# VGLoic/kzg-poly-commit-exploration

Measured on AMD Instinct MI355X. Metric: g1_msm_commitments_per_sec_degree_2^20, higher is better.
Workload: dtype i32 digits (Fp: 13 signed radix-2^30 digits, Montgomery 2^390; Fr: 8 x u32, Montgomery 2^256)

## Files before the change

### include/kzg_mi355x.h

```cpp
#ifndef KZG_MI355X_H
#define KZG_MI355X_H

#include <stddef.h>
#include <stdint.h>

#ifdef __cplusplus
extern "C" {
#endif

typedef struct kzg_ctx kzg_ctx;

#define KZG_ABI_VERSION 4
int kzg_abi_version(void);

typedef enum kzg_status {
    KZG_OK = 0,
    KZG_ERR_DEGREE_TOO_HIGH = -1,
    KZG_ERR_CONSTANT_POLY = -2,
    KZG_ERR_REMAINDER = -3,
    KZG_ERR_INVALID_ARG = -4,
    KZG_ERR_NO_DEVICE = -5,
    KZG_ERR_HIP = -6,
    KZG_ERR_NO_SRS = -7,
    KZG_ERR_BUSY = -8
// ... 478 lines not shown
                   size_t* bad_index );
int kzg_srs_verify_lincomb(kzg_ctx* ctx, const uint64_t* weights, const void* setup_g2, size_t g2_stride_bytes,
                           uint64_t out_a_p1[18], uint64_t out_b_p1[18], int* valid);

int kzg_g2_mul(const uint64_t in_p2[36], const uint8_t scalar_be[32], uint64_t out_p2[36]);
int kzg_srs_verify_update(const uint64_t before_p1[18], const uint64_t after_p1[18], const uint64_t tau_g2[36], int* valid);


typedef struct kzg_kernel_times {
    float digits_ms;
    float scatter_ms;
    float accumulate_ms;
    float reduce_ms;
    float quotient_ms;
    float total_ms;
    uint64_t references;
    float accumulate_events_ms;
    float reserved_;
} kzg_kernel_times;

int kzg_set_timing(kzg_ctx* ctx, int enabled);
int kzg_get_times(kzg_ctx* ctx, int slot, kzg_kernel_times* out);
int kzg_msm_config(const kzg_ctx* ctx, int* digit_bits, int* table_levels, size_t* num_buckets, int* recoding);

#ifdef __cplusplus
}
#endif
#endif
```

### kzg_poly_commit_exploration_amd/__init__.py

```python
import ctypes as C
import os

import numpy as np

__all__ = [
    "Engine", "Scalar", "G1Point", "Polynomial", "Evaluation", "SetupArtifactsGenerator", "KzgError",
    "R_MODULUS", "lib_path", "load_library", "ABI_SYMBOLS", "srs_g2_at", "verify_proof", "verify_proof_batch",
    "verify_points", "KZG_MAX_OPEN_POINTS", "KZG_NTT_MAX_LOG", "KZG_GP_MAX_COLUMNS", "KZG_PQ_MAX_COLUMNS", "KZG_LOGUP_MAX_COLUMNS",
    "KZG_PQ_MAX_LOG_EXT", "KZG_EXTEND_VALUES", "KZG_EXTEND_COEFFS", "domain_root",
    "Circuit", "circuit_verify", "circuit_blinders", "circuit_blinded_sizes", "circuit_proof_size", "circuit_proof_challenges", "circuit_verify_proof",
    "KZG_CIRCUIT_MIN_COLUMNS", "KZG_CIRCUIT_COL_QLIN", "KZG_CIRCUIT_COL_QM", "KZG_CIRCUIT_COL_QC", "KZG_CIRCUIT_COL_SIGMA",
    "KZG_CIRCUIT_COL_L0", "KZG_CIRCUIT_VALUES", "KZG_CIRCUIT_COEFFS", "KZG_CIRCUIT_COSET",
    "KZG_CIRCUIT_COL_TABLE", "KZG_CIRCUIT_COL_QLOOKUP",
    "circuit_lookup_proof_size", "circuit_lookup_proof_challenges", "circuit_lookup_verify_proof",
    "combine_claims", "verify_combined", "KZG_MAX_COMBINE",
    "verify_sets", "KZG_MAX_SETS", "KZG_MAX_SET_POINTS",
    "sha256", "sha256_has_shani", "blob_challenges_bytes",
]

_HERE = os.path.dirname(os.path.abspath(__file__))
R_MODULUS = 0x73EDA753299D7D483339D80809A1D80553BDA402FFFE5BFEFFFFFFFF00000001
_FR_R = 1 << 256
_FR_RINV = pow(_FR_R, -1, R_MODULUS)

KZG_OK = 0
KZG_ERR_DEGREE_TOO_HIGH = -1
KZG_ERR_CONSTANT_POLY = -2
KZG_ERR_REMAINDER = -3
KZG_ERR_INVALID_ARG = -4
KZG_ERR_NO_DEVICE = -5
KZG_ERR_HIP = -6
KZG_ERR_NO_SRS = -7
KZG_ERR_BUSY = -8
KZG_MULTI_REPLICATE_SRS = 1
KZG_ABI_VERSION = 4

ABI_SYMBOLS = [
    "kzg_ctx_create", "kzg_ctx_destroy", "kzg_strerror", "kzg_last_error",
    "kzg_srs_load_g1", "kzg_srs_generate_g1", "kzg_srs_read_g1", "kzg_srs_len",
    "kzg_commit", "kzg_commit_le_bytes", "kzg_open", "kzg_quotient", "kzg_evaluate",
    "kzg_srs_load_affine", "kzg_srs_load_compressed", "kzg_srs_save", "kzg_srs_load_file",
    "kzg_ctx_create_multi", "kzg_ctx_create_multi_ex", "kzg_abi_version", "kzg_commit_batch", "kzg_open_batch", "kzg_num_devices", "kzg_rccl_exchanges", "kzg_num_slots", "kzg_commit_submit", "kzg_open_submit", "kzg_wait",
    "kzg_set_max_batch", "kzg_max_batch", "kzg_commit_batch_submit", "kzg_wait_batch",
    "kzg_open_batch_submit", "kzg_wait_open_batch", "kzg_g1_uncompress",
    "kzg_dev_alloc", "kzg_dev_free", "kzg_dev_upload", "kzg_dev_download",
    "kzg_g1_sum", "kzg_g1_compress", "kzg_srs_g2_at", "kzg_verify_proof", "kzg_verify_proof_batch", "kzg_set_timing", "kzg_get_times", "kzg_msm_config",
    "kzg_open_points", "kzg_open_points_submit", "kzg_quotient_points", "kzg_evaluate_points", "kzg_verify_points",
    "kzg_domain_root", "kzg_ntt", "kzg_ntt_device", "kzg_commit_evaluations", "kzg_commit_evaluations_submit",
    "kzg_open_evaluations", "kzg_cells_and_proofs", "kzg_cells_and_proofs_evaluations", "kzg_quotient_cells",
    "kzg_cells_and_proofs_fk20", "kzg_fk20_prepare", "kzg_g1_dft", "kzg_recover_cells_and_proofs",
    "kzg_verify_cells_batch", "kzg_verify_cells_lincomb",
    "kzg_evaluate_evaluations_batch", "kzg_verify_openings_batch", "kzg_verify_openings_lincomb", "kzg_verify_evaluations_batch",
    "kzg_verify_cells_batch_bytes", "kzg_verify_cells_lincomb_bytes", "kzg_verify_openings_batch_bytes",
    "kzg_verify_openings_lincomb_bytes", "kzg_verify_blobs_batch_bytes", "kzg_g1_uncompress_batch", "kzg_fr_from_bytes_batch",
    "kzg_blobs_to_commitments_bytes", "kzg_blobs_to_cells_and_proofs_bytes", "kzg_recover_cells_and_proofs_bytes",
    "kzg_g1_compress_batch", "kzg_fr_to_bytes_batch",
    "kzg_srs_update", "kzg_srs_verify", "kzg_srs_verify_lincomb", "kzg_g2_mul", "kzg_srs_verify_update",
    "kzg_open_combined", "kzg_open_combined_submit", "kzg_wait_combined", "kzg_get_combine_ms", "kzg_combine_polys",
    "kzg_evaluate_batch_at", "kzg_combine_claims", "kzg_verify_combined",
    "kzg_open_sets", "kzg_open_sets_submit", "kzg_wait_sets", "kzg_quotient_sets", "kzg_verify_sets",
    "kzg_sha256", "kzg_sha256_pieces", "kzg_sha256_has_shani", "kzg_blob_challenges_bytes", "kzg_blobs_open_at_bytes", "kzg_blobs_to_blob_proofs_bytes",
    "kzg_verify_blob_proofs_batch_bytes",
    "kzg_lagrange_prepare", "kzg_lagrange_len", "kzg_lagrange_read_g1", "kzg_lagrange_load_compressed",
    "kzg_srs_load_lagrange_compressed", "kzg_commit_lagrange", "kzg_commit_lagrange_submit", "kzg_commit_lagrange_batch",
    "kzg_open_lagrange", "kzg_open_lagrange_submit", "kzg_quotient_lagrange",
    "kzg_grand_product", "kzg_grand_product_device", "kzg_permutation_product", "kzg_permutation_product_device",
    "kzg_permutation_commit",
    "kzg_logderivative_sum", "kzg_logderivative_sum_device", "kzg_lookup_sum", "kzg_lookup_sum_device", "kzg_lookup_commit",
    "kzg_batch_inverse", "kzg_batch_inverse_device", "kzg_lookup_multiplicities", "kzg_lookup_multiplicities_device",
# ... 102 lines not shown
        "kzg_num_slots": (i, [vp]),
        "kzg_commit_submit": (i, [vp, i, vp, sz]),
        "kzg_open_submit": (i, [vp, i, vp, sz, vp, vp]),
        "kzg_wait": (i, [vp, i, vp]),
        "kzg_set_max_batch": (i, [vp, sz]),
        "kzg_max_batch": (sz, [vp]),
        "kzg_commit_batch_submit": (i, [vp, i, vp, sz, sz, sz]),
        "kzg_wait_batch": (i, [vp, i, vp, sz]),
        "kzg_open_batch_submit": (i, [vp, i, vp, sz, sz, sz, vp, vp]),
        "kzg_wait_open_batch": (i, [vp, i, vp, vp, sz]),
        "kzg_g1_uncompress": (i, [u8p, vp]),
        "kzg_dev_alloc": (i, [vp, sz, C.POINTER(vp)]),
        "kzg_dev_free": (i, [vp, vp]),
        "kzg_dev_upload": (i, [vp, vp, vp, sz]),
        "kzg_dev_download": (i, [vp, vp, vp, sz]),
        "kzg_g1_sum": (i, [vp, sz, vp]),
        "kzg_g1_compress": (i, [vp, vp]),
        "kzg_set_timing": (i, [vp, i]),
        "kzg_get_times": (i, [vp, i, C.POINTER(KernelTimes)]),
        "kzg_srs_g2_at": (i, [u8p, C.c_uint64, vp]),
        "kzg_verify_proof": (i, [vp, vp, vp, vp, vp, C.POINTER(i)]),
        "kzg_verify_proof_batch": (i, [vp, vp, vp, vp, vp, sz, vp]),
        "kzg_msm_config": (i, [vp, C.POINTER(i), C.POINTER(i), C.POINTER(sz), C.POINTER(i)]),
        "kzg_open_points": (i, [vp, vp, sz, vp, vp, sz, vp]),
        "kzg_open_points_submit": (i, [vp, i, vp, sz, vp, vp, sz]),
        "kzg_quotient_points": (i, [vp, vp, sz, vp, vp, sz, vp, C.POINTER(sz)]),
        "kzg_evaluate_points": (i, [vp, vp, sz, vp, sz, vp]),
        "kzg_verify_points": (i, [vp, vp, vp, vp, sz, vp, sz, vp, sz, C.POINTER(i)]),
        "kzg_domain_root": (i, [C.c_uint, vp]),
        "kzg_ntt": (i, [vp, vp, sz, i, vp]),
        "kzg_ntt_device": (i, [vp, vp, vp, sz, i]),
        "kzg_ntt_batch": (i, [vp, vp, sz, sz, sz, i, vp, sz]),
        "kzg_ntt_batch_device": (i, [vp, vp, sz, sz, sz, vp, sz, i]),
        "kzg_ntt_batch_rounds": (i, [vp, sz, sz, C.POINTER(sz)]),
        "kzg_commit_evaluations": (i, [vp, vp, sz, vp]),
        "kzg_commit_evaluations_submit": (i, [vp, i, vp, sz]),
        "kzg_open_evaluations": (i, [vp, vp, sz, vp, vp, vp]),
        "kzg_lagrange_prepare": (i, [vp, C.c_uint]),
        "kzg_lagrange_len": (sz, [vp]),
        "kzg_lagrange_read_g1": (i, [vp, sz, sz, vp]),
        "kzg_lagrange_load_compressed": (i, [vp, vp, sz, C.c_uint, i, C.POINTER(sz), C.POINTER(i)]),
        "kzg_srs_load_lagrange_compressed": (i, [vp, vp, sz, C.c_uint, C.POINTER(sz)]),
        "kzg_commit_lagrange": (i, [vp, vp, sz, vp]),
        "kzg_commit_lagrange_submit": (i, [vp, i, vp, sz]),
        "kzg_commit_lagrange_batch": (i, [vp, vp, sz, sz, sz, vp]),
        "kzg_open_lagrange": (i, [vp, vp, sz, vp, vp, vp]),
# ... 1448 lines not shown
                for i in range(b)]

    def commit_batch_limbs(self, polys):
        polys = [np.ascontiguousarray(p, dtype=np.uint64).reshape(-1, 4) for p in polys]
        n = polys[0].shape[0]
        assert all(p.shape[0] == n for p in polys)
        flat = np.concatenate(polys)
        dptr = self.dev_alloc(flat.nbytes)
        try:
            self.dev_upload(dptr, flat)
            self.commit_batch_submit(0, dptr, n, len(polys))
            return self.wait_batch(0, len(polys))
        finally:
            self.dev_free(dptr)

    def set_timing(self, enabled):
        _check(self._lib.kzg_set_timing(self._h, 1 if enabled else 0))

    def times(self, slot):
        t = KernelTimes()
        _check(self._lib.kzg_get_times(self._h, slot, C.byref(t)))
        return {n: getattr(t, n) for n, _ in KernelTimes._fields_}


class Circuit:

    def __init__(self, engine, handle, n, t, log_ext, key):
        self._eng, self._c = engine, handle
        self.n, self.t, self.log_ext, self.key = n, t, log_ext, key
        self.c = 0
        self.g, self.exponents = 0, None
        self.rho, self.exponents_next = 0, None

    def close(self):
        if getattr(self, "_c", None) and getattr(self._eng, "_h", None):
            self._eng._pq_check(self._eng._lib.kzg_circuit_destroy(self._eng._h, self._c))
        self._c = None

    def quotient(self, wires, z, alpha, beta, gamma, public_inputs=None, gate=None, n=None, want_coeffs=True, want_commitments=True,
                 engine=None):
        e = self._eng if engine is None else engine
        a, t, stride, n = e._columns(wires, self.n if n is None else n)
        assert t == self.t and n == self.n
        zz = np.ascontiguousarray(z, dtype=np.uint64).reshape(-1, 4)
        assert zz.shape[0] >= n
        N = n << self.log_ext
# ... 692 lines not shown
```

### kzg_poly_commit_exploration_amd/csrc/api.hip

```cpp
#include <hip/hip_runtime.h>
#include <sys/random.h>

#include <algorithm>
#include <atomic>
#include <cerrno>
#include <chrono>
#include <condition_variable>
#include <cstdio>
#include <cstdlib>
#include <cstring>
#include <deque>
#include <functional>
#include <mutex>
#include <new>
#include <string>
#include <thread>
#include <vector>

#include "../../include/kzg_mi355x.h"
#include "engine.h"
#include "host_field.hpp"
#include "host_fr.hpp"
#include "fr30_host.hpp"
#include "host_pairing.hpp"
// ... 103 lines not shown

struct SlotQueue {
    hipStream_t stream = nullptr;
    hipStream_t end = nullptr;
    hipEvent_t ev[8] = {};
    hipEvent_t done = nullptr;
    hipEvent_t sorted_ev = nullptr, accum_ev = nullptr;
    hipEvent_t cmb_ev[2] = {};
    hipEvent_t cells_ev = nullptr;
    hipEvent_t upload_ev = nullptr;
    SlotQueue() = default;
    SlotQueue(const SlotQueue&) = delete;
    SlotQueue& operator=(const SlotQueue&) = delete;
    ~SlotQueue() {
        for (hipEvent_t e : {ev[0], ev[1], ev[2], ev[3], ev[4], ev[5], ev[6], ev[7], cmb_ev[0], cmb_ev[1], cells_ev, upload_ev, done, sorted_ev, accum_ev})
            if (e) hipEventDestroy(e);
    }
};

struct Slot : SlotQueue {
    DevBuf cnt, offs, block_sums, pairs, sorted, buckets;
    DevBuf recoded;
    DevBuf part_a, part_b;
    DevBuf pair_scratch;
    DevBuf heavy_ws;
    DevBuf arena;
    PinnedBuf fin{PinnedBuf::Mapped};
    DevBuf stage;
    DevBuf q;
    DevBuf chunk, block;
    PinnedBuf small{PinnedBuf::Mapped};
    PinnedBuf bsmall{PinnedBuf::Mapped};
    std::vector<uint32_t> open_ys;
    PinnedBuf roots{PinnedBuf::Staged};
    PinnedBuf pvals{PinnedBuf::Mapped};
    DevBuf pblock;
    std::vector<uint32_t> pts_ys;
    size_t pts_nq = 0;
    PinnedBuf ctab{PinnedBuf::Staged};
    PinnedBuf cvals{PinnedBuf::Mapped};
    DevBuf cpart, cin;
    size_t cmb_t = 0;
    float combine_ms = 0;
    PinnedBuf stab{PinnedBuf::Staged}, ssel{PinnedBuf::Staged};
    PinnedBuf svals{PinnedBuf::Mapped};
    DevBuf sg;
// ... 105 lines not shown

struct TmpStream {
    hipStream_t s = nullptr;
    ~TmpStream() { if (s) hipStreamDestroy(s); }
};

int sync_unlocked(kzg_ctx* ctx, std::unique_lock<std::mutex>& lk, hipStream_t st, const char* what) {
    lk.unlock();
    const hipError_t e = hipStreamSynchronize(st);
    lk.lock();
    return e == hipSuccess ? KZG_OK : hip_fail(ctx, what, e);
}
constexpr const char* kCopyCoeffs = "hipMemcpyAsync (coefficients)";
int copy_unlocked(kzg_ctx* ctx, std::unique_lock<std::mutex>& lk, hipStream_t st, void* dst, const void* src, size_t bytes,
                  hipMemcpyKind kind, const char* what) {
    if (!bytes) return KZG_OK;
    lk.unlock();
    const hipError_t e = hipMemcpyAsync(dst, src, bytes, kind, st);
    lk.lock();
    return e == hipSuccess ? KZG_OK : hip_fail(ctx, what, e);
}

void free_slot_msm(Slot& s) {
    for (DevBuf* b : {&s.cnt, &s.offs, &s.block_sums, &s.pairs, &s.recoded, &s.sorted, &s.buckets, &s.part_a, &s.part_b, &s.pair_scratch,
                      &s.heavy_ws, &s.arena})
        b->reset();
    s.fin.reset();
}

int create_stream(kzg_ctx* ctx, hipStream_t* out, bool high) {
    int least = 0, greatest = 0;
    HIP_TRY(ctx, hipDeviceGetStreamPriorityRange(&least, &greatest));
    const char* v = std::getenv("KZG_STREAM_PRIORITIES");
    const bool prio = !(v && v[0] == '0');
    HIP_TRY(ctx, hipStreamCreateWithPriority(out, hipStreamNonBlocking, prio ? (high ? greatest : least) : 0));
    return KZG_OK;
}

int ensure_slot_basics(kzg_ctx* ctx, Slot& s) {
    if (s.stream) return KZG_OK;
    if (!ctx->front_stream) {
        int rc = create_stream(ctx, &ctx->front_stream, false);
        if (rc) return rc;
    }
    if (!ctx->upload_stream) HIP_TRY(ctx, hipStreamCreateWithFlags(&ctx->upload_stream, hipStreamNonBlocking));
    for (auto& e : s.ev)
        if (!e) HIP_TRY(ctx, hipEventCreate(&e));
// ... 85 lines not shown
    const size_t pairs = (size_t)cfg.max_digits * ctx->n * B;
    for (int i = 0; i < kNumSlots; i++) {
        Slot& s = ctx->slots[i];
        {
            int rcb = ensure_slot_basics(ctx, s);
            if (rcb) return rcb;
        }
        if (!s.sorted_ev) {
            HIP_TRY(ctx, hipEventCreateWithFlags(&s.sorted_ev, hipEventDisableTiming));
            HIP_TRY(ctx, hipEventCreateWithFlags(&s.accum_ev, hipEventDisableTiming));
        }
        free_slot_msm(s);
        int rc = s.cnt.reserve(ctx, (size_t)sort_count_entries((uint32_t)B, cfg) * 4 + 64);
        if (rc == KZG_OK) rc = s.offs.reserve(ctx, ((size_t)cfg.nb * B + 1) * 4);
        if (rc == KZG_OK) rc = s.block_sums.reserve(ctx, (size_t)sort_workspace_words() * 4);
        if (rc) return rc;
        HIP_TRY(ctx, hipMemset(s.block_sums.p, 0, (size_t)sort_workspace_zero_words() * 4));
        rc = s.pairs.reserve(ctx, (pairs ? pairs : 1) * 8);
        if (rc == KZG_OK) rc = s.recoded.reserve(ctx, (ctx->n * B ? ctx->n * B : 1) * 32);
        if (rc == KZG_OK) rc = s.sorted.reserve(ctx, (pairs ? pairs : 1) * 4);
        if (rc == KZG_OK) rc = s.buckets.reserve(ctx, (size_t)cfg.nb * B * kXyzzBytes);
        if (rc == KZG_OK) rc = s.part_a.reserve(ctx, (size_t)kMaxAccumLanes * kXyzzBytes);
        if (rc == KZG_OK) rc = s.part_b.reserve(ctx, (size_t)kMaxAccumLanes * kXyzzBytes);
        if (rc == KZG_OK) rc = s.pair_scratch.reserve(ctx, accumulate_pair_scratch_bytes(pairs));
        if (rc == KZG_OK) rc = s.heavy_ws.reserve(ctx, heavy_workspace_bytes());
        if (rc == KZG_OK) rc = s.arena.reserve(ctx, ctx->arena_records * B * kXyzzBytes);
        if (rc == KZG_OK) rc = s.fin.reserve(ctx, ctx->final_records * B * kXyzzBytes);
        if (rc) return rc;
        s.kind = SLOT_IDLE;
    }
    ctx->slots_ready = true;
    return KZG_OK;
}

int build_tables(kzg_ctx* ctx, hipStream_t st, void* d_xyzz_tmp, void* d_prefix) {
    const size_t n = ctx->n;
    for (uint32_t j = 1; j < ctx->cfg.W; j++) {
        char* prev = (char*)ctx->table.p + (size_t)(j - 1) * n * kAffineBytes;
        char* next = (char*)ctx->table.p + (size_t)j * n * kAffineBytes;
        launch_table_window(st, prev, (uint32_t)n, ctx->cfg.level_bits, d_xyzz_tmp, d_prefix, next);
    }
    HIP_TRY(ctx, hipGetLastError());
    HIP_TRY(ctx, hipStreamSynchronize(st));
    return KZG_OK;
}

// ... 50 lines not shown
    if (s.timing) {
        HIP_TRY(ctx, hipEventRecord(s.ev[ev_base + 1], st));
        HIP_TRY(ctx, hipEventRecord(s.ev[ev_base + 2], st));
    }
    bool alone = true;
    for (const auto& other : ctx->slots) alone = alone && (&other == &s || other.kind == SLOT_IDLE);
    const uint64_t max_refs = (uint64_t)n * cfg.max_digits * batch;
    const uint32_t lanes = accumulate_lanes(max_refs, alone);
    const ReducePlan& P = ctx->plan;
    const uint32_t R = 1u << P.hi_bits, C = 1u << P.lo_bits, B = batch;
    char* row = (char*)s.arena.p;
    char* col = row + (size_t)R * B * kXyzzBytes;
    char* fin = (char*)s.fin.d;
    const uint32_t rl = 1u << P.row_lo, rh = 1u << P.row_hi, cl = 1u << P.col_lo, ch = 1u << P.col_hi;
    const TreeSumDesc stage1[2] = {
        {s.buckets.p, row, B * R, C, C, 1, B * R, 0},
        {s.buckets.p, col, B * C, R, 1, C, C, (uint64_t)cfg.nb}};
    const TreeSumDesc stage2[4] = {
        {row, fin + (size_t)P.off_r2row * B * kXyzzBytes, B * rh, rl, rl, 1, rh, R},
        {row, fin + (size_t)P.off_c2row * B * kXyzzBytes, B * rl, rh, 1, rl, rl, R},
        {col, fin + (size_t)P.off_r2col * B * kXyzzBytes, B * ch, cl, cl, 1, ch, C},
        {col, fin + (size_t)P.off_c2col * B * kXyzzBytes, B * cl, ch, 1, cl, cl, C}};
    if (!header_zeroed) HIP_TRY(ctx, hipMemsetAsync(s.heavy_ws.p, 0, kHeavyHeaderBytes, st));
    if (max_refs <= kTinyRefs && !ctx->small_msm_off) {
        if (s.timing) HIP_TRY(ctx, hipEventRecord(s.ev[ev_base + 3], st));
        launch_small_msm(st, table, s.sorted.dev(), s.offs.dev(), nbt, lanes, max_refs, s.buckets.p, s.part_a.p, s.part_b.p,
                         s.heavy_ws.p, s.small.dev() + 26, stage1, stage2, ctx->small_lds_bytes);
        if (s.timing) HIP_TRY(ctx, hipEventRecord(s.ev[ev_base + 4], st));
    } else {
        const bool hand_over = !alone;
        hipStream_t hs = hand_over ? ctx->heavy_stream : st;
        if (hand_over) {
            HIP_TRY(ctx, hipEventRecord(s.sorted_ev, st));
            HIP_TRY(ctx, hipStreamWaitEvent(hs, s.sorted_ev, 0));
        }
        if (s.timing) HIP_TRY(ctx, hipEventRecord(s.ev[ev_base + 3], hs));
        launch_bucket_accumulate(hs, table, s.sorted.dev(), s.offs.dev(), nbt, lanes, s.buckets.p, s.part_a.p, s.part_b.p,
                                 ctx->accum_lds_bytes, s.pair_scratch.p, max_refs,
                                 (char*)s.heavy_ws.p + kAccumClockOffset);
        if (s.timing) HIP_TRY(ctx, hipEventRecord(s.ev[ev_base + 4], hs));
        if (hand_over) {
            HIP_TRY(ctx, hipEventRecord(s.accum_ev, hs));
            st = s.end = ctx->tail_stream;
            HIP_TRY(ctx, hipStreamWaitEvent(st, s.accum_ev, 0));
        }
        launch_bucket_finalize(st, s.offs.dev(), nbt, lanes, s.part_a.p, s.part_b.p, s.buckets.p, s.heavy_ws.p, s.small.dev() + 26,
                               finalize_group_size(nbt));
        launch_tree_sums_two_stage(st, stage1, 2, stage2, 4, (uint32_t*)s.heavy_ws.p + 64, alone);
    }
    if (s.timing) HIP_TRY(ctx, hipEventRecord(s.ev[ev_base + 5], st));
    HIP_TRY(ctx, hipGetLastError());
    return KZG_OK;
}

hf::PX host_wsum(const uint64_t* recs, uint32_t len) {
    hf::PX run = hf::px_inf(), acc = hf::px_inf();
    for (uint32_t v = len; v-- > 1;) {
        run = hf::px_add(run, hf::px_from_record(recs + (size_t)v * kXyzzWords64));
        acc = hf::px_add(acc, run);
    }
// ... 9432 lines not shown
    std::memcpy(&before, before_p1, sizeof before);
    std::memcpy(&after, after_p1, sizeof after);
    if (before.is_inf() || after.is_inf() || !hf::p1_on_curve(before) || !hf::p1_on_curve(after)) return KZG_OK;
    if (q.inf || !g2_in_subgroup(tau_g2)) return KZG_OK;
    *valid = vc_pair(before_p1, after_p1, q, hf::g2_generator());
    return KZG_OK;
}


int kzg_set_timing(kzg_ctx* ctx, int enabled) {
    KZG_SINGLE_DEVICE_ONLY(ctx);
    if (!ctx) return KZG_ERR_INVALID_ARG;
    std::lock_guard<std::mutex> lk(ctx->mu);
    ctx->timing = enabled != 0;
    return KZG_OK;
}
int kzg_get_times(kzg_ctx* ctx, int slot, kzg_kernel_times* out) {
    KZG_SINGLE_DEVICE_ONLY(ctx);
    if (!ctx || !out || slot < 0 || slot >= kNumSlots) return KZG_ERR_INVALID_ARG;
    std::lock_guard<std::mutex> lk(ctx->mu);
    *out = ctx->slots[slot].times;
    return KZG_OK;
}

}
```

### kzg_poly_commit_exploration_amd/csrc/engine.h

```cpp
#pragma once
#include <hip/hip_runtime.h>
#include <stddef.h>
#include <stdint.h>

namespace kzg {

constexpr size_t kAffineBytes = 128;
constexpr size_t kAffineU4 = kAffineBytes / 16;
constexpr size_t kXyzzBytes = 256;
constexpr size_t kXyzzU4 = kXyzzBytes / 16;
constexpr size_t kXyzzWords64 = kXyzzBytes / 8;

enum : uint32_t { kRecodeWindows = 0, kRecodeNaf = 1 };
struct MsmConfig {
    uint32_t recode;
    uint32_t c;
    uint32_t W;
    uint32_t level_bits;
    uint32_t nb;
    uint32_t max_digits;
};

MsmConfig choose_msm_config(size_t n_points, size_t table_budget_bytes);

constexpr uint32_t kTinyRefs = 65536;
__host__ __device__ inline uint32_t accumulate_min_seg(uint64_t refs) { return refs <= kTinyRefs ? 4u : 8u; }
__host__ __device__ inline uint32_t accumulate_seg_len(uint32_t M, uint32_t lanes) {
    uint32_t L = (M + lanes - 1) / lanes;
    const uint32_t lo = accumulate_min_seg(M);
    return L < lo ? lo : L;
}

constexpr size_t kHeavyHeaderBytes = 1024;
uint32_t sort_count_entries(uint32_t max_batch, MsmConfig cfg);
uint32_t sort_max_batch(MsmConfig cfg);
uint32_t sort_workspace_words();
uint32_t sort_workspace_zero_words();
bool launch_bucket_sort(hipStream_t s, const uint32_t* d_scalars, int scalars_are_mont, uint32_t n, uint32_t batch,
                        uint64_t stride, uint32_t table_stride, MsmConfig cfg, uint32_t* d_cnt,
                        uint32_t* d_ws, uint64_t* d_pairs, uint32_t* d_recoded, uint32_t* d_offs, uint32_t* d_sorted,
                        uint32_t* d_header);
constexpr uint32_t kMaxAccumLanes = 262144 + 64;
uint32_t accumulate_lanes(uint64_t max_refs, bool alone = false);
size_t accumulate_pair_scratch_bytes(uint64_t max_refs);
void launch_bucket_accumulate(hipStream_t s, const void* d_table, const uint32_t* d_sorted, const uint32_t* d_offs,
                              uint32_t nb, uint32_t lanes, void* d_buckets ,
                              void* d_part_a, void* d_part_b, uint32_t lds_reserve_bytes, void* d_pair_scratch,
                              uint64_t max_refs, void* d_clock = nullptr );
constexpr size_t kAccumClockOffset = 768;
size_t heavy_workspace_bytes();
void launch_bucket_finalize(hipStream_t s, const uint32_t* d_offs, uint32_t nb, uint32_t lanes, const void* d_part_a,
                            const void* d_part_b, void* d_buckets, void* d_heavy_ws,
                            uint32_t* d_refs_out , uint32_t group = 1);
uint32_t finalize_group_size(uint32_t nb);
struct TreeSumDesc;
uint32_t small_msm_lds_bytes();
const void* small_msm_kernel();
void launch_small_msm(hipStream_t s, const void* d_table, const uint32_t* d_sorted, const uint32_t* d_offs, uint32_t nb,
                      uint32_t lanes, uint64_t max_refs, void* d_buckets, void* d_part_a, void* d_part_b, void* d_heavy_ws,
                      uint32_t* d_refs_out, const TreeSumDesc* stage1 , const TreeSumDesc* stage2 ,
                      uint32_t lds_bytes);
struct TreeSumDesc {
    const void* in;
    void* out;
    uint32_t groups, len;
    uint64_t gstride, estride;
    uint32_t inner;
    uint64_t ostride;
// ... 329 lines not shown
```

### kzg_poly_commit_exploration_amd/csrc/msm_accum.hip

```cpp
#include <cstdlib>

#ifndef KZG_ACCUM_PARALLEL_COLUMNS
#define KZG_F30_SERIAL_COLUMNS 1
#endif
#include "engine.h"
#include "field30_inv.hip.h"
#include "g1_30.hip.h"

namespace kzg {

#ifndef KZG_ACCUM_BLOCK
#define KZG_ACCUM_BLOCK 256
#endif
constexpr int kAccumBlock = KZG_ACCUM_BLOCK;

__device__ __forceinline__ Fq load_fq(const uint4* __restrict__ p) {
    const uint4 a = p[0], b = p[1], c = p[2];
    const uint32_t d = reinterpret_cast<const uint32_t*>(p)[12];
    Fq r;
    r.d[0] = (int32_t)a.x; r.d[1] = (int32_t)a.y; r.d[2] = (int32_t)a.z; r.d[3] = (int32_t)a.w;
    r.d[4] = (int32_t)b.x; r.d[5] = (int32_t)b.y; r.d[6] = (int32_t)b.z; r.d[7] = (int32_t)b.w;
    r.d[8] = (int32_t)c.x; r.d[9] = (int32_t)c.y; r.d[10] = (int32_t)c.z; r.d[11] = (int32_t)c.w;
    r.d[12] = (int32_t)d;
    return r;
}
__device__ __forceinline__ Affine30 load_affine30(const uint4* __restrict__ table, uint32_t idx) {
    const uint4* p = table + (size_t)idx * kAffineU4;
    Affine30 r;
    r.x = load_fq(p);
    r.y = load_fq(p + 4);
    return r;
}

__device__ __forceinline__ uint32_t bucket_of(const uint32_t* __restrict__ offs, uint32_t nb, uint32_t pos) {
    uint32_t lo = 0, hi = nb;
    while (hi - lo > 1) {
        uint32_t mid = (lo + hi) >> 1;
        if (offs[mid] <= pos) lo = mid; else hi = mid;
    }
    return lo;
}

typedef __attribute__((address_space(3))) char* lds_char_ptr;
typedef uint32_t accum_u32x4 __attribute__((ext_vector_type(4)));
typedef const __attribute__((address_space(3))) accum_u32x4* lds_u4_ptr;
extern __shared__ uint4 lds_points[];
__device__ __forceinline__ uint32_t accum_wave_lane() { return __builtin_amdgcn_mbcnt_hi(~0u, __builtin_amdgcn_mbcnt_lo(~0u, 0u)); }
__device__ __forceinline__ uint32_t accum_wave_slot() {
    const uint32_t lds0 = (uint32_t)(uintptr_t)(lds_char_ptr)(char*)lds_points;
    return lds0 + __builtin_amdgcn_readfirstlane(threadIdx.x >> 6) * (8u * 64u * 16u);
}
__device__ __forceinline__ void accum_issue_gather(const uint4* __restrict__ table, uint32_t slot, uint32_t r) {
    const char* src = reinterpret_cast<const char*>(table + (size_t)(r & 0x7fffffffu) * kAffineU4);
#pragma unroll
    for (int k = 0; k < 8; k++)
        __builtin_amdgcn_global_load_lds((const __attribute__((address_space(1))) void*)(src + 16 * k),
                                         (__attribute__((address_space(3))) void*)(lds_char_ptr)(uintptr_t)(slot + 1024u * k),
                                         16, 0, 0);
}
constexpr int kFlushOps = 17;
static_assert(kFlushOps == 17, "the literal in accum_take_point's s_waitcnt");
__device__ __forceinline__ Affine30 accum_read_point(uint32_t lane_slot) {
    Affine30 r;
// ... 46 lines not shown
        "global_store_dwordx4 %0, %8, off offset:112\n\t"
        "global_store_dwordx4 %0, %9, off offset:128\n\t"
        "global_store_dwordx4 %0, %10, off offset:144\n\t"
        "global_store_dwordx4 %0, %11, off offset:160\n\t"
        "global_store_dwordx4 %0, %12, off offset:176\n\t"
        "global_store_dwordx4 %0, %13, off offset:192\n\t"
        "global_store_dwordx4 %0, %14, off offset:208\n\t"
        "global_store_dwordx4 %0, %15, off offset:224\n\t"
        "global_store_dwordx4 %0, %16, off offset:240"
        :
        : "v"(dst), "v"(v[0]), "v"(v[1]), "v"(v[2]), "v"(v[3]), "v"(v[4]), "v"(v[5]), "v"(v[6]), "v"(v[7]), "v"(v[8]), "v"(v[9]),
          "v"(v[10]), "v"(v[11]), "v"(v[12]), "v"(v[13]), "v"(v[14]), "v"(v[15])
        : "memory");
}
__device__ __forceinline__ uint32_t accum_ref(const uint32_t* __restrict__ sorted, uint32_t i) {
    return *reinterpret_cast<const uint32_t*>(reinterpret_cast<const char*>(sorted) + (uint32_t)(i * 4u));
}

#ifndef KZG_ACCUM_MIN_BLOCKS
#define KZG_ACCUM_MIN_BLOCKS 2
#endif
__global__ void __launch_bounds__(kAccumBlock, KZG_ACCUM_MIN_BLOCKS)
k_bucket_accumulate(const uint4* __restrict__ table, const uint32_t* __restrict__ sorted, const uint32_t* __restrict__ offs,
                    uint32_t nb, uint32_t lanes, uint4* __restrict__ buckets, uint4* __restrict__ part_a,
                    uint4* __restrict__ part_b, unsigned long long* __restrict__ clk) {
    asm volatile("" ::: "v175");
    const bool stamp = clk != nullptr && (threadIdx.x & 63) == 0;
    if (stamp) atomicMax(&clk[0], ~(unsigned long long)wall_clock64());
    const uint32_t lane = blockIdx.x * kAccumBlock + threadIdx.x;
    const uint32_t M = offs[nb];
    const uint32_t L = accumulate_seg_len(M, lanes);
    const uint64_t start64 = (uint64_t)lane * L;
    if (start64 >= M) return;
    const uint32_t start = (uint32_t)start64;
    const uint32_t end = (M - start < L) ? M : start + L;

    uint32_t b = bucket_of(offs, nb, start);
    uint32_t b_beg = offs[b], b_end = offs[b + 1];
    uint32_t b_end_next = offs[(b + 2 <= nb) ? b + 2 : nb];
    uint32_t run_start = start;
    XYZZ30 acc = xyzz30_inf();
    const uint32_t wave_slot = accum_wave_slot();
    uint32_t ref = accum_ref(sorted, start);
    uint32_t ref_next = accum_ref(sorted, min(start + 1, M - 1));
    accum_issue_gather(table, wave_slot, ref);
    for (uint32_t e = start; e < end; e++) {
        const bool wave_flushed = __builtin_amdgcn_ballot_w64(e == b_end) != 0;
        if (e == b_end) {
            uint4* dst = (run_start == b_beg) ? buckets + (size_t)b * kXyzzU4 : part_a + (size_t)lane * kXyzzU4;
            xyzz30_acc_settle(acc);
            accum_flush_run(dst, acc);
            acc = xyzz30_inf();
            b++;
            b_beg = b_end;
            b_end = b_end_next;
            while (b_end <= e) {
                b++;
                b_beg = b_end;
                b_end = offs[b + 1];
            }
            b_end_next = offs[(b + 2 <= nb) ? b + 2 : nb];
            run_start = e;
        }
        Fq P, Rn;
        uint32_t code;
        {
            const Affine30 p = accum_take_point(wave_slot, wave_flushed);
            code = xyzz30_acc_head(acc, p, (ref >> 31) != 0, P, Rn);
        }
        bool more = code == 0;
        if (__builtin_amdgcn_ballot_w64(code != 0) != 0) {
            if (code & kAccFresh) {
                if (!(code & kAccPointInf)) {
                    const Affine30 p = accum_read_point(wave_slot + accum_wave_lane() * 16u);
                    xyzz30_acc_set(acc, p, (ref >> 31) != 0);
                }
            } else if (code == kAccMaybeEqual) {
                AccumRare t;
                t.acc = acc;
                t.P = P;
                t.Rn = Rn;
                more = accum_rare_call(&t);
                acc = t.acc;
                P = t.P;
                Rn = t.Rn;
                __builtin_amdgcn_s_waitcnt(0x0f70);
            }
        }
        ref = ref_next;
        if (e + 1 < end) accum_issue_gather(table, wave_slot, ref);
        ref_next = accum_ref(sorted, min(e + 2, M - 1));
        if (more) xyzz30_acc_tail(acc, P, Rn);
    }
    uint4* dst;
    if (run_start == b_beg && end == b_end) dst = buckets + (size_t)b * kXyzzU4;
    else if (run_start == start) dst = part_a + (size_t)lane * kXyzzU4;
    else dst = part_b + (size_t)lane * kXyzzU4;
    xyzz30_acc_settle(acc);
    store_xyzz30(dst, acc);
    if (stamp) atomicMax(&clk[1], (unsigned long long)wall_clock64());
}

constexpr uint32_t kPairRecU4 = 4;

static __device__ __noinline__ Fq fq_mul_call(Fq a, Fq b) { return fq_mul(a, b); }
static __device__ __noinline__ Fq fq_sqr_call(Fq a) { return fq_sqr(a); }
#ifdef KZG_PAIR_CALLS
#define KZG_PAIR_MUL(a, b) fq_mul_call(a, b)
#define KZG_PAIR_SQR(a) fq_sqr_call(a)
#else
#define KZG_PAIR_MUL(a, b) fq_mul(a, b)
#define KZG_PAIR_SQR(a) fq_sqr(a)
#endif
static __device__ __noinline__ void fq_inv_call(Fq* io) {
    const Fq a = *io;
    *io = fq_inv(a);
}
static __device__ __noinline__ uint32_t pair_classify_call(const Affine30* a, bool nega, const Affine30* b, bool negb, Fq* den) {
    Fq d;
    const uint32_t kind = pair_classify(*a, nega, *b, negb, d);
// ... 216 lines not shown
        uint64_t l = v ? std::strtoull(v, nullptr, 10) : 131072ull;
        return l < 64 ? 131072ull : (l > 262144ull ? 262144ull : l);
    }();
    const uint64_t lo = accumulate_min_seg(max_refs);
    uint64_t lanes = (max_refs + lo - 1) / lo;
    if (lanes > target) lanes = target;
    lanes = (lanes + kAccumBlock - 1) / kAccumBlock * kAccumBlock;
    return (uint32_t)lanes;
}

bool accumulate_pairs_enabled() {
    static const int pairs_mode = [] {
        const char* v = std::getenv("KZG_ACCUM_PAIRS");
        return v ? std::atoi(v) : 0;
    }();
    return pairs_mode != 0;
}
size_t accumulate_pair_scratch_bytes(uint64_t max_refs) {
    if (!accumulate_pairs_enabled()) return 0;
    return (size_t)(max_refs / 2 + kMaxAccumLanes) * kPairRecU4 * 16;
}

void launch_bucket_accumulate(hipStream_t s, const void* d_table, const uint32_t* d_sorted, const uint32_t* d_offs,
                              uint32_t nb, uint32_t lanes, void* d_buckets, void* d_part_a, void* d_part_b,
                              uint32_t lds_reserve_bytes, void* d_pair_scratch, uint64_t max_refs, void* d_clock) {
    if (!lanes) return;
    if (accumulate_pairs_enabled() && d_pair_scratch && max_refs / lanes >= 16) {
        hipLaunchKernelGGL(k_bucket_accumulate_pairs, dim3(lanes / kAccumBlock), dim3(kAccumBlock),
                           (kAccumBlock / 64) * 16 * 64 * 16 , s,
                           reinterpret_cast<const uint4*>(d_table), d_sorted, d_offs, nb, lanes,
                           reinterpret_cast<uint4*>(d_buckets), reinterpret_cast<uint4*>(d_part_a),
                           reinterpret_cast<uint4*>(d_part_b), reinterpret_cast<uint4*>(d_pair_scratch));
        return;
    }
    const uint32_t need = (kAccumBlock / 64) * 8 * 64 * 16;
    lds_reserve_bytes = lds_reserve_bytes / (256 / kAccumBlock);
    if (lds_reserve_bytes < need) lds_reserve_bytes = need;
    hipLaunchKernelGGL(k_bucket_accumulate, dim3(lanes / kAccumBlock), dim3(kAccumBlock), lds_reserve_bytes, s,
                       reinterpret_cast<const uint4*>(d_table), d_sorted, d_offs, nb, lanes,
                       reinterpret_cast<uint4*>(d_buckets), reinterpret_cast<uint4*>(d_part_a),
                       reinterpret_cast<uint4*>(d_part_b), reinterpret_cast<unsigned long long*>(d_clock));
}

}
```

### kzg_poly_commit_exploration_amd/csrc/msm_sort.hip

```cpp
#include <cstdlib>
#include <cstring>
#include <type_traits>

#include "engine.h"
#include "fr30.hip.h"
#include "msm_recode.h"

namespace kzg {

typedef uint32_t u32;
#ifndef KZG_DEV
#define KZG_DEV __device__ __forceinline__
#endif

static uint32_t ilog2(uint32_t v) {
    uint32_t b = 0;
    while ((1u << b) < v) b++;
    return b;
}

MsmConfig choose_msm_config(size_t n, size_t table_budget_bytes) {
    const char* force_mode = std::getenv("KZG_MSM_RECODE");
    const char* force_c = std::getenv("KZG_MSM_C");
    const uint32_t fc = force_c ? (uint32_t)std::strtoul(force_c, nullptr, 10) : 0u;
// ... 47 lines not shown
    k[0] = lo.x, k[1] = lo.y, k[2] = lo.z, k[3] = lo.w, k[4] = hi.x, k[5] = hi.y, k[6] = hi.z, k[7] = hi.w;
    return recode_unpack(k);
}

template <uint32_t C, class F>
KZG_DEV void for_each_digit(const u32 k[8], MsmConfig cfg, F&& f) {
    if constexpr (C != 0) {
        for_each_window_digit_fixed<C>(k, f);
    } else if (cfg.recode == kRecodeNaf) {
        for_each_naf_digit(k, cfg.c, f);
    } else {
        u32 t[8];
#pragma unroll
        for (int w = 0; w < 8; w++) t[w] = k[w];
        for_each_window_digit(t, cfg.c, cfg.W, f);
    }
}
static uint32_t fixed_width(MsmConfig cfg) {
    return cfg.recode == kRecodeWindows && (cfg.c == 15 || cfg.c == 16 || cfg.c == 17 || cfg.c == 19) ? cfg.c : 0u;
}

constexpr int kSortBlock = 256;
constexpr int kRecodeBlock = 512;
#ifndef KZG_SORT_TILES
#define KZG_SORT_TILES 512
#endif
constexpr uint32_t kMaxTiles = KZG_SORT_TILES;
constexpr int kMaxCoarse = 2048;
constexpr int kFineMax = 256;

struct SortGeom {
    uint32_t tile;
    uint32_t tiles;
    uint32_t fine_bits;
    uint32_t coarse_bins;
    bool packed;
};

constexpr uint32_t kPackedFineBits = 7, kPackedIndexBits = 24;
static uint32_t sort_fine_bits(MsmConfig cfg, bool packed) {
    const uint32_t bits = ilog2(cfg.nb), most = packed ? kPackedFineBits : 8u;
    return bits < most ? bits : most;
}
static bool sort_packed_buckets(uint32_t nb_total, MsmConfig cfg);

static bool sort_packed_buckets(uint32_t nb_total, MsmConfig cfg) { return (nb_total >> sort_fine_bits(cfg, true)) <= (uint32_t)kMaxCoarse; }
// ... 593 lines not shown
```

Baseline: 442.2.

## Reorder accumulate lanes by first bucket-boundary position to reduce wave divergence

Adds a two-kernel planning pass that computes each accumulation segment's starting bucket once, keys it by where its first bucket boundary falls, and counting-sorts segments by that key. The accumulate kernel then reads its segment and bucket from the plan, so lanes in a wave hit bucket flushes at similar iterations, and the per-lane binary search is gone. The accumulator reset on a flush now clears only ZZ, with the full reset moved into the infinity case. This costs two small extra launches and a plan buffer, and it adds a debug API for reading the plan.

```diff
diff --git a/include/kzg_mi355x.h b/include/kzg_mi355x.h
--- a/include/kzg_mi355x.h
+++ b/include/kzg_mi355x.h
@@ -524,6 +524,8 @@
 int kzg_set_timing(kzg_ctx* ctx, int enabled);
 int kzg_get_times(kzg_ctx* ctx, int slot, kzg_kernel_times* out);
 int kzg_msm_config(const kzg_ctx* ctx, int* digit_bits, int* table_levels, size_t* num_buckets, int* recoding);
+int kzg_get_accum_plan(kzg_ctx* ctx, int slot, uint32_t* lanes, uint32_t* buckets, uint32_t* plan, size_t plan_words,
+                       uint32_t* offs, size_t offs_words);
 
 #ifdef __cplusplus
 }
diff --git a/kzg_poly_commit_exploration_amd/__init__.py b/kzg_poly_commit_exploration_amd/__init__.py
--- a/kzg_poly_commit_exploration_amd/__init__.py
+++ b/kzg_poly_commit_exploration_amd/__init__.py
@@ -44,7 +44,7 @@
     "kzg_set_max_batch", "kzg_max_batch", "kzg_commit_batch_submit", "kzg_wait_batch",
     "kzg_open_batch_submit", "kzg_wait_open_batch", "kzg_g1_uncompress",
     "kzg_dev_alloc", "kzg_dev_free", "kzg_dev_upload", "kzg_dev_download",
-    "kzg_g1_sum", "kzg_g1_compress", "kzg_srs_g2_at", "kzg_verify_proof", "kzg_verify_proof_batch", "kzg_set_timing", "kzg_get_times", "kzg_msm_config",
+    "kzg_g1_sum", "kzg_g1_compress", "kzg_srs_g2_at", "kzg_verify_proof", "kzg_verify_proof_batch", "kzg_set_timing", "kzg_get_times", "kzg_msm_config", "kzg_get_accum_plan",
     "kzg_open_points", "kzg_open_points_submit", "kzg_quotient_points", "kzg_evaluate_points", "kzg_verify_points",
     "kzg_domain_root", "kzg_ntt", "kzg_ntt_device", "kzg_commit_evaluations", "kzg_commit_evaluations_submit",
     "kzg_open_evaluations", "kzg_cells_and_proofs", "kzg_cells_and_proofs_evaluations", "kzg_quotient_cells",
@@ -193,6 +193,7 @@
         "kzg_verify_proof": (i, [vp, vp, vp, vp, vp, C.POINTER(i)]),
         "kzg_verify_proof_batch": (i, [vp, vp, vp, vp, vp, sz, vp]),
         "kzg_msm_config": (i, [vp, C.POINTER(i), C.POINTER(i), C.POINTER(sz), C.POINTER(i)]),
+        "kzg_get_accum_plan": (i, [vp, i, C.POINTER(C.c_uint32), C.POINTER(C.c_uint32), vp, sz, vp, sz]),
         "kzg_open_points": (i, [vp, vp, sz, vp, vp, sz, vp]),
         "kzg_open_points_submit": (i, [vp, i, vp, sz, vp, vp, sz]),
         "kzg_quotient_points": (i, [vp, vp, sz, vp, vp, sz, vp, C.POINTER(sz)]),
@@ -1687,6 +1688,15 @@
         _check(self._lib.kzg_get_times(self._h, slot, C.byref(t)))
         return {n: getattr(t, n) for n, _ in KernelTimes._fields_}
 
+    def accum_plan(self, slot):
+        lanes, buckets = C.c_uint32(), C.c_uint32()
+        _check(self._lib.kzg_get_accum_plan(self._h, slot, C.byref(lanes), C.byref(buckets), None, 0, None, 0))
+        plan = np.zeros((lanes.value, 2), dtype=np.uint32)
+        offs = np.zeros(buckets.value + 1, dtype=np.uint32)
+        _check(self._lib.kzg_get_accum_plan(self._h, slot, C.byref(lanes), C.byref(buckets), plan.ctypes.data_as(C.c_void_p), plan.size,
+                                            offs.ctypes.data_as(C.c_void_p), offs.size))
+        return (plan if lanes.value else None), offs
+
 
 class Circuit:
 
diff --git a/kzg_poly_commit_exploration_amd/csrc/api.hip b/kzg_poly_commit_exploration_amd/csrc/api.hip
--- a/kzg_poly_commit_exploration_amd/csrc/api.hip
+++ b/kzg_poly_commit_exploration_amd/csrc/api.hip
@@ -149,6 +149,8 @@
     DevBuf cnt, offs, block_sums, pairs, sorted, buckets;
     DevBuf recoded;
     DevBuf part_a, part_b;
+    DevBuf plan;
+    uint32_t plan_lanes = 0, plan_buckets = 0;
     DevBuf pair_scratch;
     DevBuf heavy_ws;
     DevBuf arena;
@@ -300,7 +302,7 @@
 }
 
 void free_slot_msm(Slot& s) {
-    for (DevBuf* b : {&s.cnt, &s.offs, &s.block_sums, &s.pairs, &s.recoded, &s.sorted, &s.buckets, &s.part_a, &s.part_b, &s.pair_scratch,
+    for (DevBuf* b : {&s.cnt, &s.offs, &s.block_sums, &s.pairs, &s.recoded, &s.sorted, &s.buckets, &s.part_a, &s.part_b, &s.plan, &s.pair_scratch,
                       &s.heavy_ws, &s.arena})
         b->reset();
     s.fin.reset();
@@ -432,6 +434,7 @@
         if (rc == KZG_OK) rc = s.buckets.reserve(ctx, (size_t)cfg.nb * B * kXyzzBytes);
         if (rc == KZG_OK) rc = s.part_a.reserve(ctx, (size_t)kMaxAccumLanes * kXyzzBytes);
         if (rc == KZG_OK) rc = s.part_b.reserve(ctx, (size_t)kMaxAccumLanes * kXyzzBytes);
+        if (rc == KZG_OK) rc = s.plan.reserve(ctx, kAccumPlanBytes);
         if (rc == KZG_OK) rc = s.pair_scratch.reserve(ctx, accumulate_pair_scratch_bytes(pairs));
         if (rc == KZG_OK) rc = s.heavy_ws.reserve(ctx, heavy_workspace_bytes());
         if (rc == KZG_OK) rc = s.arena.reserve(ctx, ctx->arena_records * B * kXyzzBytes);
@@ -528,6 +531,8 @@
         {col, fin + (size_t)P.off_r2col * B * kXyzzBytes, B * ch, cl, cl, 1, ch, C},
         {col, fin + (size_t)P.off_c2col * B * kXyzzBytes, B * cl, ch, 1, cl, cl, C}};
     if (!header_zeroed) HIP_TRY(ctx, hipMemsetAsync(s.heavy_ws.p, 0, kHeavyHeaderBytes, st));
+    s.plan_lanes = 0;
+    s.plan_buckets = nbt;
     if (max_refs <= kTinyRefs && !ctx->small_msm_off) {
         if (s.timing) HIP_TRY(ctx, hipEventRecord(s.ev[ev_base + 3], st));
         launch_small_msm(st, table, s.sorted.dev(), s.offs.dev(), nbt, lanes, max_refs, s.buckets.p, s.part_a.p, s.part_b.p,
@@ -536,12 +541,14 @@
     } else {
         const bool hand_over = !alone;
         hipStream_t hs = hand_over ? ctx->heavy_stream : st;
+        launch_accum_plan(st, s.offs.dev(), nbt, lanes, (uint32_t*)((char*)s.heavy_ws.p + kAccumPlanBinsOffset), s.plan.p);
+        s.plan_lanes = lanes;
         if (hand_over) {
             HIP_TRY(ctx, hipEventRecord(s.sorted_ev, st));
             HIP_TRY(ctx, hipStreamWaitEvent(hs, s.sorted_ev, 0));
         }
         if (s.timing) HIP_TRY(ctx, hipEventRecord(s.ev[ev_base + 3], hs));
-        launch_bucket_accumulate(hs, table, s.sorted.dev(), s.offs.dev(), nbt, lanes, s.buckets.p, s.part_a.p, s.part_b.p,
+        launch_bucket_accumulate(hs, table, s.sorted.dev(), s.offs.dev(), s.plan.p, nbt, lanes, s.buckets.p, s.part_a.p, s.part_b.p,
                                  ctx->accum_lds_bytes, s.pair_scratch.p, max_refs,
                                  (char*)s.heavy_ws.p + kAccumClockOffset);
         if (s.timing) HIP_TRY(ctx, hipEventRecord(s.ev[ev_base + 4], hs));
@@ -10020,5 +10027,25 @@
     *out = ctx->slots[slot].times;
     return KZG_OK;
 }
-
-}
+int kzg_get_accum_plan(kzg_ctx* ctx, int slot, uint32_t* lanes, uint32_t* buckets, uint32_t* plan, size_t plan_words, uint32_t* offs,
+                       size_t offs_words) {
+    KZG_SINGLE_DEVICE_ONLY(ctx);
+    if (!ctx || !lanes || !buckets || slot < 0 || slot >= kNumSlots) return KZG_ERR_INVALID_ARG;
+    std::lock_guard<std::mutex> lk(ctx->mu);
+    Slot& s = ctx->slots[slot];
+    if (!ctx->slots_ready || s.kind != SLOT_IDLE) return KZG_ERR_INVALID_ARG;
+    HIP_TRY(ctx, hipSetDevice(ctx->device));
+    *lanes = s.plan_lanes;
+    *buckets = s.plan_buckets;
+    if (plan && s.plan_lanes) {
+        if (plan_words < 2 * (size_t)s.plan_lanes) return KZG_ERR_INVALID_ARG;
+        HIP_TRY(ctx, hipMemcpy(plan, s.plan.p, (size_t)s.plan_lanes * 8, hipMemcpyDeviceToHost));
+    }
+    if (offs && s.plan_buckets) {
+        if (offs_words < (size_t)s.plan_buckets + 1) return KZG_ERR_INVALID_ARG;
+        HIP_TRY(ctx, hipMemcpy(offs, s.offs.p, ((size_t)s.plan_buckets + 1) * 4, hipMemcpyDeviceToHost));
+    }
+    return KZG_OK;
+}
+
+}
diff --git a/kzg_poly_commit_exploration_amd/csrc/engine.h b/kzg_poly_commit_exploration_amd/csrc/engine.h
--- a/kzg_poly_commit_exploration_amd/csrc/engine.h
+++ b/kzg_poly_commit_exploration_amd/csrc/engine.h
@@ -31,7 +31,7 @@
     return L < lo ? lo : L;
 }
 
-constexpr size_t kHeavyHeaderBytes = 1024;
+constexpr size_t kHeavyHeaderBytes = 2048;
 uint32_t sort_count_entries(uint32_t max_batch, MsmConfig cfg);
 uint32_t sort_max_batch(MsmConfig cfg);
 uint32_t sort_workspace_words();
@@ -43,7 +43,10 @@
 constexpr uint32_t kMaxAccumLanes = 262144 + 64;
 uint32_t accumulate_lanes(uint64_t max_refs, bool alone = false);
 size_t accumulate_pair_scratch_bytes(uint64_t max_refs);
-void launch_bucket_accumulate(hipStream_t s, const void* d_table, const uint32_t* d_sorted, const uint32_t* d_offs,
+constexpr size_t kAccumPlanBinsOffset = 1024;
+constexpr size_t kAccumPlanBytes = (size_t)kMaxAccumLanes * 8 * 2;
+void launch_accum_plan(hipStream_t s, const uint32_t* d_offs, uint32_t nb, uint32_t lanes, uint32_t* d_bins, void* d_plan);
+void launch_bucket_accumulate(hipStream_t s, const void* d_table, const uint32_t* d_sorted, const uint32_t* d_offs, const void* d_plan,
                               uint32_t nb, uint32_t lanes, void* d_buckets ,
                               void* d_part_a, void* d_part_b, uint32_t lds_reserve_bytes, void* d_pair_scratch,
                               uint64_t max_refs, void* d_clock = nullptr );
diff --git a/kzg_poly_commit_exploration_amd/csrc/msm_accum.hip b/kzg_poly_commit_exploration_amd/csrc/msm_accum.hip
--- a/kzg_poly_commit_exploration_amd/csrc/msm_accum.hip
+++ b/kzg_poly_commit_exploration_amd/csrc/msm_accum.hip
@@ -6,6 +6,7 @@
 #include "engine.h"
 #include "field30_inv.hip.h"
 #include "g1_30.hip.h"
+#include "msm_accum_plan.h"
 
 namespace kzg {
 
@@ -32,13 +33,71 @@
     return r;
 }
 
-__device__ __forceinline__ uint32_t bucket_of(const uint32_t* __restrict__ offs, uint32_t nb, uint32_t pos) {
-    uint32_t lo = 0, hi = nb;
-    while (hi - lo > 1) {
-        uint32_t mid = (lo + hi) >> 1;
-        if (offs[mid] <= pos) lo = mid; else hi = mid;
-    }
-    return lo;
+constexpr int kPlanBlock = 256;
+static_assert(kPlanBlock == (int)kPlanBins, "lane t of a workgroup owns key t");
+static_assert(kMaxAccumLanes < (1u << 24), "a position inside a key shares a word with the key");
+static_assert(kAccumPlanBinsOffset + kPlanBins * 4 <= kHeavyHeaderBytes, "the key counters lie in the job's zeroed header");
+
+__global__ void __launch_bounds__(kPlanBlock) k_accum_plan_count(const uint32_t* __restrict__ offs, uint32_t nb, uint32_t lanes,
+                                                                 uint32_t* __restrict__ bins ,
+                                                                 uint2* __restrict__ tmp) {
+    __shared__ uint32_t s_hist[kPlanBins];
+    const uint32_t t = threadIdx.x, seg = blockIdx.x * kPlanBlock + t;
+    s_hist[t] = 0;
+    __syncthreads();
+    const uint32_t M = offs[nb];
+    const uint32_t L = accumulate_seg_len(M, lanes);
+    const uint64_t start64 = (uint64_t)seg * L;
+    const bool live = seg < lanes && start64 < M;
+    uint32_t b = 0, key = 0, rank = 0;
+    if (live) {
+        const uint32_t start = (uint32_t)start64;
+        const uint32_t end = (M - start < L) ? M : start + L;
+        b = bucket_of(offs, nb, start);
+        key = accum_plan_key(start, end, offs[b + 1], accum_plan_shift(L));
+        rank = atomicAdd(&s_hist[key], 1u);
+    }
+    __syncthreads();
+    const uint32_t mine = s_hist[t];
+    __syncthreads();
+    s_hist[t] = mine ? atomicAdd(&bins[t], mine) : 0u;
+    __syncthreads();
+    if (live) tmp[seg] = make_uint2(b, key | ((s_hist[key] + rank) << 8));
+}
+
+__global__ void __launch_bounds__(kPlanBlock) k_accum_plan_place(uint32_t lanes, const uint32_t* __restrict__ bins,
+                                                                 const uint2* __restrict__ tmp, uint2* __restrict__ plan) {
+    __shared__ uint32_t s_scan[kPlanBins];
+    const uint32_t t = threadIdx.x, seg = blockIdx.x * kPlanBlock + t;
+    const uint32_t mine = bins[t];
+    s_scan[t] = mine;
+    __syncthreads();
+    for (uint32_t off = 1; off < kPlanBins; off <<= 1) {
+        const uint32_t add = t >= off ? s_scan[t - off] : 0u;
+        __syncthreads();
+        s_scan[t] += add;
+        __syncthreads();
+    }
+    const uint32_t live = s_scan[kPlanBins - 1];
+    __syncthreads();
+    s_scan[t] -= mine;
+    __syncthreads();
+    if (seg >= lanes) return;
+    if (seg < live) {
+        const uint2 r = tmp[seg];
+        plan[s_scan[r.y & (kPlanBins - 1)] + (r.y >> 8)] = make_uint2(seg, r.x);
+    } else {
+        plan[seg] = make_uint2(kPlanDead, 0u);
+    }
+}
+
+void launch_accum_plan(hipStream_t s, const uint32_t* d_offs, uint32_t nb, uint32_t lanes, uint32_t* d_bins, void* d_plan) {
+    if (!lanes) return;
+    uint2* plan = reinterpret_cast<uint2*>(d_plan);
+    uint2* tmp = plan + kMaxAccumLanes;
+    const uint32_t groups = (lanes + kPlanBlock - 1) / kPlanBlock;
+    hipLaunchKernelGGL(k_accum_plan_count, dim3(groups), dim3(kPlanBlock), 0, s, d_offs, nb, lanes, d_bins, tmp);
+    hipLaunchKernelGGL(k_accum_plan_place, dim3(groups), dim3(kPlanBlock), 0, s, lanes, (const uint32_t*)d_bins, (const uint2*)tmp, plan);
 }
 
 typedef __attribute__((address_space(3))) char* lds_char_ptr;
@@ -131,20 +190,20 @@
 #endif
 __global__ void __launch_bounds__(kAccumBlock, KZG_ACCUM_MIN_BLOCKS)
 k_bucket_accumulate(const uint4* __restrict__ table, const uint32_t* __restrict__ sorted, const uint32_t* __restrict__ offs,
-                    uint32_t nb, uint32_t lanes, uint4* __restrict__ buckets, uint4* __restrict__ part_a,
-                    uint4* __restrict__ part_b, unsigned long long* __restrict__ clk) {
+                    const uint2* __restrict__ plan, uint32_t nb, uint32_t lanes, uint4* __restrict__ buckets,
+                    uint4* __restrict__ part_a, uint4* __restrict__ part_b, unsigned long long* __restrict__ clk) {
     asm volatile("" ::: "v175");
     const bool stamp = clk != nullptr && (threadIdx.x & 63) == 0;
     if (stamp) atomicMax(&clk[0], ~(unsigned long long)wall_clock64());
-    const uint32_t lane = blockIdx.x * kAccumBlock + threadIdx.x;
+    const uint2 mine = plan[blockIdx.x * kAccumBlock + threadIdx.x];
+    const uint32_t seg = mine.x;
+    if (seg == kPlanDead) return;
     const uint32_t M = offs[nb];
     const uint32_t L = accumulate_seg_len(M, lanes);
-    const uint64_t start64 = (uint64_t)lane * L;
-    if (start64 >= M) return;
-    const uint32_t start = (uint32_t)start64;
+    const uint32_t start = seg * L;
     const uint32_t end = (M - start < L) ? M : start + L;
 
-    uint32_t b = bucket_of(offs, nb, start);
+    uint32_t b = mine.y;
     uint32_t b_beg = offs[b], b_end = offs[b + 1];
     uint32_t b_end_next = offs[(b + 2 <= nb) ? b + 2 : nb];
     uint32_t run_start = start;
@@ -156,10 +215,10 @@
     for (uint32_t e = start; e < end; e++) {
         const bool wave_flushed = __builtin_amdgcn_ballot_w64(e == b_end) != 0;
         if (e == b_end) {
-            uint4* dst = (run_start == b_beg) ? buckets + (size_t)b * kXyzzU4 : part_a + (size_t)lane * kXyzzU4;
+            uint4* dst = (run_start == b_beg) ? buckets + (size_t)b * kXyzzU4 : part_a + (size_t)seg * kXyzzU4;
             xyzz30_acc_settle(acc);
             accum_flush_run(dst, acc);
-            acc = xyzz30_inf();
+            acc.ZZ = fq_zero();
             b++;
             b_beg = b_end;
             b_end = b_end_next;
@@ -183,6 +242,8 @@
                 if (!(code & kAccPointInf)) {
                     const Affine30 p = accum_read_point(wave_slot + accum_wave_lane() * 16u);
                     xyzz30_acc_set(acc, p, (ref >> 31) != 0);
+                } else {
+                    acc = xyzz30_inf();
                 }
             } else if (code == kAccMaybeEqual) {
                 AccumRare t;
@@ -203,8 +264,8 @@
     }
     uint4* dst;
     if (run_start == b_beg && end == b_end) dst = buckets + (size_t)b * kXyzzU4;
-    else if (run_start == start) dst = part_a + (size_t)lane * kXyzzU4;
-    else dst = part_b + (size_t)lane * kXyzzU4;
+    else if (run_start == start) dst = part_a + (size_t)seg * kXyzzU4;
+    else dst = part_b + (size_t)seg * kXyzzU4;
     xyzz30_acc_settle(acc);
     store_xyzz30(dst, acc);
     if (stamp) atomicMax(&clk[1], (unsigned long long)wall_clock64());
@@ -467,7 +528,7 @@
 }
 
 void launch_bucket_accumulate(hipStream_t s, const void* d_table, const uint32_t* d_sorted, const uint32_t* d_offs,
-                              uint32_t nb, uint32_t lanes, void* d_buckets, void* d_part_a, void* d_part_b,
+                              const void* d_plan, uint32_t nb, uint32_t lanes, void* d_buckets, void* d_part_a, void* d_part_b,
                               uint32_t lds_reserve_bytes, void* d_pair_scratch, uint64_t max_refs, void* d_clock) {
     if (!lanes) return;
     if (accumulate_pairs_enabled() && d_pair_scratch && max_refs / lanes >= 16) {
@@ -482,7 +543,7 @@
     lds_reserve_bytes = lds_reserve_bytes / (256 / kAccumBlock);
     if (lds_reserve_bytes < need) lds_reserve_bytes = need;
     hipLaunchKernelGGL(k_bucket_accumulate, dim3(lanes / kAccumBlock), dim3(kAccumBlock), lds_reserve_bytes, s,
-                       reinterpret_cast<const uint4*>(d_table), d_sorted, d_offs, nb, lanes,
+                       reinterpret_cast<const uint4*>(d_table), d_sorted, d_offs, reinterpret_cast<const uint2*>(d_plan), nb, lanes,
                        reinterpret_cast<uint4*>(d_buckets), reinterpret_cast<uint4*>(d_part_a),
                        reinterpret_cast<uint4*>(d_part_b), reinterpret_cast<unsigned long long*>(d_clock));
 }
diff --git a/kzg_poly_commit_exploration_amd/csrc/msm_accum_plan.h b/kzg_poly_commit_exploration_amd/csrc/msm_accum_plan.h
--- /dev/null
+++ b/kzg_poly_commit_exploration_amd/csrc/msm_accum_plan.h
@@ -0,0 +1,37 @@
+#pragma once
+#include <stdint.h>
+
+#ifndef KZG_HD
+#ifdef __HIPCC__
+#define KZG_HD __host__ __device__ __forceinline__
+#else
+#define KZG_HD inline
+#endif
+#endif
+
+namespace kzg {
+
+constexpr uint32_t kPlanBins = 256;
+constexpr uint32_t kPlanNoEnd = kPlanBins - 1;
+constexpr uint32_t kPlanDead = 0xffffffffu;
+
+KZG_HD uint32_t bucket_of(const uint32_t* offs, uint32_t nb, uint32_t pos) {
+    uint32_t lo = 0, hi = nb;
+    while (hi - lo > 1) {
+        uint32_t mid = (lo + hi) >> 1;
+        if (offs[mid] <= pos) lo = mid; else hi = mid;
+    }
+    return lo;
+}
+
+KZG_HD uint32_t accum_plan_shift(uint32_t L) {
+    uint32_t s = 0;
+    while (((L - 1) >> s) >= kPlanNoEnd) s++;
+    return s;
+}
+
+KZG_HD uint32_t accum_plan_key(uint32_t start, uint32_t end, uint32_t b_end, uint32_t shift) {
+    return b_end < end ? (b_end - start) >> shift : kPlanNoEnd;
+}
+
+}
diff --git a/kzg_poly_commit_exploration_amd/csrc/msm_sort.hip b/kzg_poly_commit_exploration_amd/csrc/msm_sort.hip
--- a/kzg_poly_commit_exploration_amd/csrc/msm_sort.hip
+++ b/kzg_poly_commit_exploration_amd/csrc/msm_sort.hip
@@ -93,6 +93,7 @@
 
 constexpr int kSortBlock = 256;
 constexpr int kRecodeBlock = 512;
+static_assert(kHeavyHeaderBytes / 4 <= (size_t)kRecodeBlock, "workgroup 0 of k_sort_count zeroes the job's header, one word per lane");
 #ifndef KZG_SORT_TILES
 #define KZG_SORT_TILES 512
 #endif
```

Result: slower. 430.6 (-2.6%).
